# popgenmethods/smcpp

Measured on AMD Instinct MI355X. Metric: E-step loglik-evals/sec (100 Mbp, M=64, n=20), higher is better.
Workload: dtype f64 state + f32 scans (mixed)

## Files before the change

### smcpp_amd/csrc/engine_capi.hpp

```cpp
#define API_BEGIN try {
#define API_END                                                                    \
    return 0;                                                                      \
    }                                                                              \
    catch (const std::exception &e) { g_err = e.what(); return 1; }               \
    catch (...) { g_err = "unknown error"; return 1; }

extern "C" {

const char *smcpp_last_error(void) { return g_err.c_str(); }

int smcpp_create_onepop(int n, int n_contigs, const int *Ls, const int *const *obs, int n_hs, const double *hs,
                        double polarization_error, int device, smcpp_im **out) {
    API_BEGIN
    std::unique_ptr<smcpp_im> im(new smcpp_im());
    const int nn[1] = {n}, nna[1] = {2};
    im->build(1, nn, nna, n_contigs, Ls, obs, n_hs, hs, polarization_error, device);
    *out = im.release();
    API_END
}

int smcpp_create_twopop(int n1, int n2, int a1, int a2, int n_contigs, const int *Ls, const int *const *obs,
                        int n_hs, const double *hs, double polarization_error, int device, smcpp_im **out) {
    API_BEGIN
    if (a1 == 0 && a2 == 2) throw std::runtime_error("(0,2) not supported");
// ... 64 lines not shown
int smcpp_set_prep_mode(smcpp_im *im, int host) {
    API_BEGIN
    im->force_host_prep = host != 0;
    im->params_fresh = false;
    im->dirty = true;
    API_END
}

int smcpp_set_warm_start(smcpp_im *im, int on) {
    API_BEGIN
    im->warm_start = on != 0;
    if (!on) im->warm_valid = false;
    API_END
}

int smcpp_set_raw(smcpp_im *im, const double *pi, const double *T, int K, const int *keys, const double *E) {
    API_BEGIN
    const int M = im->M, kl = im->keylen;
    std::map<std::vector<int>, int> given;
    for (int k = 0; k < K; ++k) given[std::vector<int>(keys + (size_t)k * kl, keys + (size_t)(k + 1) * kl)] = k;
    std::vector<double> Enew((size_t)im->K * M);
    for (int k = 0; k < im->K; ++k) {
        std::vector<int> key(im->keys.begin() + (size_t)k * kl, im->keys.begin() + (size_t)(k + 1) * kl);
        auto it = given.find(key);
        if (it == given.end()) throw std::runtime_error("set_raw: an observed key has no emission vector");
        std::memcpy(&Enew[(size_t)k * M], E + (size_t)it->second * M, sizeof(double) * M);
    }
    im->pi.assign(pi, pi + M);
    im->T.assign(T, T + (size_t)M * M);
    im->E.swap(Enew);
    im->raw_keys.assign(keys, keys + (size_t)K * kl);
    im->raw_E.assign(E, E + (size_t)K * M);
    im->have_raw = true;
    im->E_on_dev = false;
    im->tgen_valid = false; im->dT_valid = true; im->T_lazy = false;
    im->dirty = true;
    im->nder = 0;
    API_END
}

int smcpp_estep(smcpp_im *im, int fb_only) {
    API_BEGIN
    (void)fb_only;
    im->estep();
    API_END
}

int smcpp_loglik(smcpp_im *im, double *out) {
    API_BEGIN
    std::memcpy(out, im->loglik.data(), sizeof(double) * im->n_contigs);
    API_END
}

static double dcs(const std::vector<double> &x) {
    if (x.empty()) return 0.0;
    double s = x[0], c = 0.0;
    for (size_t i = 1; i < x.size(); ++i) {
        const double y = c + x[i];
        const double u = x[i] - (y - c);
        const double t = y + s;
        const double v = y - (t - s);
        const double z = u + v;
        s = t + z;
        c = z - (s - t);
    }
    return s;
// ... 261 lines not shown
    return cols;
}
int smcpp_get_emission(smcpp_im *im, double *out, double *jac) {
    API_BEGIN
    need_model_params(im);
    im->sync_host_E();
    if (im->emission.size() != (size_t)im->M * smcpp_num_emission_cols(im)) throw std::runtime_error("emission matrix is not available");
    std::memcpy(out, im->emission.data(), sizeof(double) * im->emission.size());
    if (jac && im->nder > 0) std::memcpy(jac, im->demission.data(), sizeof(double) * im->demission.size());
    API_END
}

void smcpp_init_logger_cb(void (*cb)(const char *, const char *, const char *)) { g_logger_cb = cb; }

int smcpp_init_cache(const char *path) {
    API_BEGIN
    smcpp_host::csfs_cache_prefix() = path ? path : "";
    API_END
}

int smcpp_set_global_keys(smcpp_im *im, int Kg, const int *gkeys) {
    API_BEGIN
    const int kl = im->keylen;
    std::map<std::vector<int>, int> gm;
    for (int k = 0; k < Kg; ++k) gm[std::vector<int>(gkeys + (size_t)k * kl, gkeys + (size_t)(k + 1) * kl)] = k;
    im->local_to_global.assign(im->K, -1);
    for (int k = 0; k < im->K; ++k) {
        auto it = gm.find(std::vector<int>(im->keys.begin() + (size_t)k * kl, im->keys.begin() + (size_t)(k + 1) * kl));
        if (it == gm.end()) throw std::runtime_error("global key list misses a local key");
        im->local_to_global[k] = it->second;
    }
    im->gkeys.assign(gkeys, gkeys + (size_t)Kg * kl);
    im->have_global = true;
    im->pack_tables_ready = false;
    if (im->dprep) im->dprep->keys_ready = false;
    if (im->qdev) im->qdev->stats_ready = false;
    im->E_on_dev = false;
    im->params_fresh = false;
    im->Eg.clear(); im->dEg.clear();
    API_END
}

int smcpp_pack_stats(smcpp_im *im, double *buf, long *n_out, int dev) {
    API_BEGIN
    const int M = im->M, K = im->K;
    const int Kg = im->have_global ? (int)(im->gkeys.size() / im->keylen) : K;
    const long n = 1 + M + (long)M * M + (long)Kg * M;
    if (n_out) *n_out = n;
    if (!buf) return 0;
    if (dev && !im->estep_done) throw std::runtime_error("no E-step has been run on this manager yet");
    if (dev) {
        HIPCHK(hipSetDevice(im->device));
        if (!im->pack_tables_ready) {
            std::vector<int> g2l(Kg, -1);
            for (int k = 0; k < K; ++k) g2l[im->have_global ? im->local_to_global[k] : k] = k;
            im->d_g2l.upload(g2l, im->stream);
            im->d_present.upload(im->present, im->stream);
            HIPCHK(hipStreamSynchronize(im->stream));
            im->pack_tables_ready = true;
        }
        PackArgs pa;
        pa.M = M; pa.Mp = im->Mp; pa.K = K; pa.Kg = Kg; pa.n_contigs = im->n_contigs;
        pa.loglik = im->d_loglik.p; pa.gamma0 = im->d_gamma0.p; pa.xisum = im->d_xisum.p; pa.gsum = im->d_gsum.p;
        pa.present = im->d_present.p; pa.g2l = im->d_g2l.p; pa.out = buf;
        hipLaunchKernelGGL(k_pack_stats, dim3((unsigned)((n + 255) / 256)), dim3(256), 0, im->stream, pa);
        HIPCHK(hipGetLastError());
// ... 41 lines not shown
```

### smcpp_amd/csrc/engine_manager.hpp

```cpp
struct smcpp_im {
    int npop = 1, keylen = 3, M = 0, Mp = 0, NPL = 1, NT = 1, n_contigs = 0, K = 0, G = 0, Ke = 0;
    int n[2] = {0, 0}, na[2] = {2, 0};
    double polarization_error = 0.5;
    std::vector<double> hs;
    std::unique_ptr<smcpp_host::TwoPopPrep> twopop_prep;
    std::unique_ptr<TwoPopDevCsfs> twopop_dev;
    std::vector<int> keys;
    std::vector<int> Ls;
    std::vector<long long> contig_base;
    long long total_rows = 0;
    std::vector<RowInfo> rowinfo;
    std::vector<Group> groups;
    std::vector<int> eig_kid;
    std::vector<int> eig_of_key;
    std::vector<unsigned char> present;
    std::vector<double> span_sum;
    std::vector<double> pi_default;
    std::vector<unsigned char> key_nbpos;
    std::vector<Chunk> chunks;
    int max_chunks_per_contig = 1;
    int user_rows_per_chunk = 0;
    std::vector<int> perm1, perme;
    std::vector<int2> perm1k;
    std::vector<Slab> slabs_sc, slabs_rk, slabs_eg;
// ... 62 lines not shown
        size_t in_cap = 0;
        double *h_out = nullptr;
        size_t h_out_cap = 0;
        bool stats_ready = false;
        int Kq = 0;
        ~QDev() { if (d_in) (void)hipFree(d_in); if (h_out) (void)hipHostFree(h_out); }
    };
    std::unique_ptr<QDev> qdev;
    bool q_device(double val[4], double *jac);
    void ensure_dT();
    bool ss_static = false;
    bool ss_hybrid = false;
    bool ss_halo = false;
    int ss_hyb_th = 0x7fffffff;
    static constexpr int SS_HYB_COST = 8;
    long long ss_row_cost(int span) const { return (ss_hybrid && span > ss_hyb_th) ? SS_HYB_COST : span; }
    bool ss_dirsplit = false;
    int ss_nk_lds = 0, ss_ekey_of_slot[4] = {0, 1, 2, 3}, ss_eslot_of_key[4] = {0, 1, 2, 3};
    size_t ss_tab_bytes() const { return ss_hybrid ? ((size_t)ss_nk_lds * (ss_dirsplit ? 2 : 4) * Mp * (Mp + 1) + 8 * 64) * sizeof(double) : 0; }
    bool ss_active = false;
    bool eigfree = false;
    int ss_max_span = 0;
    int ss_nlds = 0;
    int ss_wpc = 1;
    bool ss_mid = false;
    int ss_wg_waves = 4;
    int ss_launched = 0, last_ss_passes = 0;
    bool ss_need_cert_pass = false;
    long long ss_positions = 0;
    int ss_light_f = 0, ss_light_b = 0;
    bool ss_warm_valid = false;
    bool arena_side = false;
    int ss_warm_parity = 0, ss_pass0 = 0;
    std::vector<int> ss_slot_of_key;
    DevBuf<int2> d_rowdesc_ss;
    bool split_spans = false;
    std::vector<int> user_Ls;
    std::vector<std::vector<int>> split_store, piece_row;
    std::vector<const int *> split_ptr;
    std::vector<DevBuf<int>> d_piece_first;
    DevBuf<double> d_gamma_user;
    const double *merged_gamma(int c);
    std::vector<GPiece> gp_pieces;
    std::vector<GTile> gp_tiles;
    std::vector<int> gp_pfirst;
    bool gp_built = false, gamma_pieces_last = false;
    DevBuf<GPiece> d_gp_pieces;
    DevBuf<GTile> d_gp_tiles;
    DevBuf<int> d_gp_pfirst;
    DevBuf<float> d_gp_pvf;
    DevBuf<double> d_gp_pvb, d_gp_pgam, d_gp_cs, d_gp_l2d, d_gp_gen;
    long long gp_count = -1;
    long long gamma_piece_count();
    void build_gamma_pieces();
    bool ss_generators_only();
    DevBuf<float> d_gpark;
    DevBuf<double> d_Fall;
    SsArgs ss_args;
    std::vector<Chunk> chunks_b;
    std::vector<int> ss_tasks;
    DevBuf<Chunk> d_chunks_b;
    DevBuf<int> d_tasks;
    void update_pi_default();
    bool debug = false;
    void upload_chunk_state();
    bool ss_extract_generators();
// ... 55 lines not shown
    int h_flags_cap = 0, h_ll_cap = 0;
    size_t param_cap = 0;
    int llblk = 64;
    int ZS = 8;
    int ZG = 1;
    int max_pass = 0;
    int last_fwd_passes = 0, last_bwd_passes = 0;
    float eps_f = 2e-6f;
    double eps_b = 1e-6;
    std::vector<double> loglik, h_xisum, h_gsum, h_gamma0;
    bool stats_on_host = false;
    double timing[9] = {0};
    double host_timing[4] = {0};
    std::vector<int> gkeys;
    std::vector<int> local_to_global;
    bool have_global = false;
    std::vector<double> g_stats;
    bool have_reduced = false;
    std::vector<double> Eg, dEg;
    std::vector<int> raw_keys;
    std::vector<double> raw_E;
    void global_emissions();

    ~smcpp_im() {
        if (stream) {
            for (auto &e : ev) (void)hipEventDestroy(e);
            (void)hipStreamDestroy(stream);
            if (stream2) (void)hipStreamDestroy(stream2);
            if (stream3) (void)hipStreamDestroy(stream3);
            if (stream_hi) (void)hipStreamDestroy(stream_hi);
        }
        if (d_param) (void)hipFree(d_param);
        if (d_pre) (void)hipFree(d_pre);
        if (h_flags) (void)hipHostFree(h_flags);
        if (h_ll) (void)hipHostFree(h_ll);
        if (h_done) (void)hipHostFree(h_done);
    }

    void build(int npop_, const int *nn, const int *nna, int n_contigs_, const int *Ls_, const int *const *obs,
               int n_hs, const double *hs_, double pol, int dev);
    void make_chunks();
    void make_slabs();
    void alloc_device();
    void host_prep_and_upload();
    void stage_static_and_prepass();
    void setup_power();
    ChainArgs chain_args();
    void run_chains();
    void run_stats();
    void enqueue_stats();
    void finish_stats();
    bool stats_enqueued = false;
    void estep();
    void fetch_stats();
    void prepare_params();
};

void smcpp_im::build(int npop_, const int *nn, const int *nna, int n_contigs_, const int *Ls_,
                     const int *const *obs, int n_hs, const double *hs_, double pol, int dev) {
    npop = npop_;
    keylen = 3 * npop;
    for (int p = 0; p < npop; ++p) { n[p] = nn[p]; na[p] = nna[p]; }
    polarization_error = pol;
    if (n_contigs_ <= 0) throw std::runtime_error("Observations list is empty");
    if (n_hs < 2) throw std::runtime_error("need at least two hidden state boundaries");
    hs.assign(hs_, hs_ + n_hs);
    for (int i = 1; i < n_hs; ++i)
        if (!(hs[i] >= hs[i - 1])) throw std::runtime_error("Hidden states must be in ascending order");
    M = n_hs - 1;
    Mp = (M + 15) / 16 * 16;
    NPL = M > 512 ? 16 : M > 256 ? 8 : (M + 63) / 64;
    NT = Mp / 16;
    if (M > 1024) throw std::runtime_error("M > 1024 hidden states is not supported by this build");
    n_contigs = n_contigs_;
    Ls.assign(Ls_, Ls_ + n_contigs);
    user_Ls = Ls;
    {
        const int ncol_ = 1 + keylen;
// ... 333 lines not shown
    long long rows = total_rows - n_contigs;
    int lc = user_rows_per_chunk;
    if (lc <= 0) {
        lc = opt().i(smcpp_opt::O_ROWS_PER_CHUNK, lc);
    }
    if (lc <= 0) lc = (int)std::max<long long>(512, (rows + slots - 1) / slots);
    chunks.clear();
    max_chunks_per_contig = 1;
    for (int c = 0; c < n_contigs; ++c) {
        const int L = Ls[c];
        const int nc = std::max(1, ceil_div(L, lc));
        max_chunks_per_contig = std::max(max_chunks_per_contig, nc);
        for (int j = 0; j < nc; ++j) {
            Chunk ch;
            ch.base = contig_base[c];
            ch.r0 = (int)((long long)L * j / nc);
            ch.r1 = (int)((long long)L * (j + 1) / nc);
            ch.contig = c;
            ch.first = (j == 0);
            ch.last = (j == nc - 1);
            ch.pad = 0;
            ch.h0 = ch.h1 = ch.r0;
            chunks.push_back(ch);
        }
    }
    max_pass = max_chunks_per_contig + 3;
    if (ss_static) max_pass += 4 + 2;
    chunks_b = chunks;
    for (Chunk &cb : chunks_b) cb.h0 = cb.h1 = cb.r1;
    ss_halo = false;
}

void smcpp_im::upload_chunk_state() {
    ss_warm_valid = false;
    const size_t nch = std::max(chunks.size(), chunks_b.size());
    d_chunks.upload(chunks, stream);
    d_chunks_b.upload(chunks_b, stream);
    {
        const size_t nf = chunks.size(), nb = chunks_b.size();
        ss_tasks.clear();
        size_t i = 0, j = 0;
        if (ss_hybrid && ss_dirsplit) {
            const size_t W = (size_t)ss_wg_waves;
            while (i < nf || j < nb) {
                const bool take_f = j >= nb || (i < nf && (double)i * (double)nb <= (double)j * (double)nf);
                for (size_t q = 0; q < W; ++q) {
                    if (take_f) ss_tasks.push_back(i < nf ? (int)i++ : -1);
                    else ss_tasks.push_back(j < nb ? ((1 << 30) | (int)j++) : -1);
                }
            }
        } else
        while (i < nf || j < nb) {
            const bool take_f = j >= nb || (i < nf && (double)i * (double)nb <= (double)j * (double)nf);
            if (take_f) ss_tasks.push_back((int)i++);
            else ss_tasks.push_back((1 << 30) | (int)j++);
        }
        while (ss_tasks.size() % ss_wg_waves) ss_tasks.push_back(-1);
        d_tasks.upload(ss_tasks, stream);
    }
    d_ends_f.alloc(2 * nch * Mp); d_used_f.alloc(nch * Mp);
    d_ends_b.alloc(2 * nch * Mp); d_used_b.alloc(nch * Mp);
    d_changed_f.alloc(max_pass + 1); d_changed_b.alloc(max_pass + 1);
    HIPCHK(hipStreamSynchronize(stream));
}

void smcpp_im::update_pi_default() {
    pi_default.assign(M, 0.0);
// ... 295 lines not shown
```

### smcpp_amd/csrc/engine_options.hpp

```cpp
#pragma once

namespace smcpp_opt {

enum OptId {
    O_HOST_TRACE, O_HOST_TIMING, O_OMP_BLOCKTIME, O_DUAL_STREAM, O_EVENT_FLAGS, O_LOCK_MIN_ROWS, O_CHAIN, O_SS, O_HYBRID, O_HYB_TH,
    O_COOP_BPC, O_ROWS_PER_CHUNK, O_SS_WPC, O_SS_HALO, O_HALO_LF, O_HALO_DF, O_HALO_LB, O_HALO_DB, O_SS_FWD_SHARE, O_STATS_TEAM,
    O_SLAB_ROWS, O_POWER_PREPASS, O_PREP, O_Q, O_EIG_TEAM, O_EIG_PIN, O_BWD_PRIO, O_COOP_TAB, O_POWER_DEBUG, O_BWD_PRIO_MASK,
    O_DEBUG_CYCLES, O_SS_H32, O_SS_MIXED, O_SS_LIGHT_F, O_SS_LIGHT_B, O_SS_CERT_PASS, O_POLL, O_SPEC_GAMMA, O_GAMMA_SIDE,
    O_STATS_VARIANT, O_SPAN_SCAN, O_S1_FUSE, O_EIGFREE, O_CSFS_DIRECT, O_RANK_WIDE, O_GAMMA_SCAN, O_GAMMA_PIECES, O_SPLIT_SPANS, O_T_LAZY, O_DEBUG_POISON, O_DEBUG_POISON_ONLY, O_DEBUG_POISON_LOG, O_COUNT
};

struct OptDef { const char *name, *help; };

static const OptDef OPT_DEFS[O_COUNT] = {
    {"SMCPP_HOST_TRACE",     "> 0: print a timestamped trace of the host phase of every E-step to stderr"},
    {"SMCPP_HOST_TIMING",    "set: print the split of the cold preparation / eigensolver / joint CSFS to stderr"},
    {"SMCPP_OMP_BLOCKTIME",  "libomp block time in ms (default 0; two-population managers 2)"},
    {"SMCPP_DUAL_STREAM",    "0: statistics branches on one stream"},
    {"SMCPP_EVENT_FLAGS",    "hipEventCreateWithFlags flags (default hipEventDisableSystemFence; 0 = default events)"},
    {"SMCPP_LOCK_MIN_ROWS",  "rows per (CU x 16) from which the lock-step MFMA chains are selected"},
    {"SMCPP_CHAIN",          "lock | dense | ss: force a chain family"},
    {"SMCPP_SS",             "0: no scan chains (the dense families)"},
    {"SMCPP_HYBRID",         "0: no hybrid rows on un-binned data (dense chains)"},
    {"SMCPP_HYB_TH",         "span above which a row is one eigen-power step (default 6)"},
    {"SMCPP_COOP_BPC",       "workgroups per CU of the cooperative chains"},
    {"SMCPP_ROWS_PER_CHUNK", "rows per chunk (0 = automatic)"},
    {"SMCPP_SS_WPC",         "wavefronts per SIMD of the scan chains (1..4; default by input size: M <= 64 two from 1.95, three from 12 million positions)"},
    {"SMCPP_SS_HALO",        "1 / 0: force / forbid the halo pass of the scan chains (default: M > 64, and M <= 64 with 1.35 - 12 million positions)"},
    {"SMCPP_HALO_LF",        "float halo positions, forward (2800)"},
    {"SMCPP_HALO_DF",        "exact halo positions, forward (800)"},
    {"SMCPP_HALO_LB",        "float halo positions, backward (3900)"},
    {"SMCPP_HALO_DB",        "exact halo positions, backward (1100)"},
    {"SMCPP_SS_FWD_SHARE",   "share of the wavefronts given to the forward chain"},
    {"SMCPP_STATS_TEAM",     "0: one rank partial per slab instead of per team of four"},
    {"SMCPP_SLAB_ROWS",      "minimum rows per statistics slab (128)"},
    {"SMCPP_POWER_PREPASS",  "0 / 1: eigen-free pre-pass of the dense chains off / forced"},
    {"SMCPP_PREP",           "host: the whole cold preparation on host threads"},
    {"SMCPP_Q",              "host: Q and its gradient on the host"},
    {"SMCPP_EIG_TEAM",       "threads per eigen key of the host eigensolver"},
    {"SMCPP_EIG_PIN",        "0: do not pin eigensolver teams to one L3 domain"},
    {"SMCPP_BWD_PRIO",       "s_setprio of the backward cooperative chain (0..3, default 1)"},
    {"SMCPP_COOP_TAB",       "0: test hook, tables of the cooperative chains from global memory"},
    {"SMCPP_POWER_DEBUG",    "debug level of the pre-pass"},
    {"SMCPP_BWD_PRIO_MASK",  "bit mask of the passes that raise the backward chain's priority (7)"},
    {"SMCPP_DEBUG_CYCLES",   "set: shader clocks / positions of chunk 1, pass 0 to stderr"},
    {"SMCPP_SS_H32",         "0: no two-row form of the scans at M <= 32"},
    {"SMCPP_SS_MIXED",       "0: fp64 scans in the stored passes; 1: float scans (default, one state per lane)"},
    {"SMCPP_SS_LIGHT_F",     "number of float history passes, forward"},
    {"SMCPP_SS_LIGHT_B",     "number of float history passes, backward"},
    {"SMCPP_SS_CERT_PASS",   "1: launch the all-skip certificate pass up front"},
    {"SMCPP_POLL",           "0: hipStreamSynchronize instead of polling the pinned completion word"},
    {"SMCPP_SPEC_GAMMA",     "0: save_gamma E-steps wait for the certificate before the statistics"},
    {"SMCPP_GAMMA_SIDE",     "0: per-row gammas on the main stream"},
    {"SMCPP_STATS_VARIANT",  "bit mask of stream arrangements of the statistics phase"},
    {"SMCPP_SPAN_SCAN",      "0: span fold on the matrix cores (k_span_big) instead of the scans"},
    {"SMCPP_S1_FUSE",        "0 / 1: two-kernel / one-pass span-1 statistics"},
    {"SMCPP_EIGFREE",        "0: eigensystem statistics even where the eigen-free form applies"},
    {"SMCPP_CSFS_DIRECT",    "set: literal O(pieces^2 n^2) conditioned SFS (test hook)"},
    {"SMCPP_RANK_WIDE",      "0: rank updates at M > 128 without the LDS-staged operand rows (k_rank_acc instead of k_rank_acc_wide); 4: four wavefronts per workgroup instead of eight"},
    {"SMCPP_GAMMA_SCAN",     "0: save_gamma E-steps take the eigensystem statistics and per-row gammas (M <= 256) instead of the eigen-free scans"},
    {"SMCPP_GAMMA_PIECES",   "0: per-row gammas of long rows at 64 < M <= 256 from the eigensystem (k_gamma_rows_eig) instead of eigen-power pieces + scan steps"},
    {"SMCPP_SPLIT_SPANS",    "0: rows of binned data longer than 64 positions are not cut into pieces (M > 64); 2: un-binned rows are cut as well at M <= 256 (test switch)"},
    {"SMCPP_T_LAZY",         "0: the model path expands the M x M transition matrix before the chains start and takes their generators from it (rounds 3-5)"},
    {"SMCPP_DEBUG_POISON",   "byte value every fresh device allocation is filled with (255: NaN / -1): a kernel that reads memory it was "
                             "never given shows up as NaN in a fresh process instead of depending on what the allocator recycles"},
    {"SMCPP_DEBUG_POISON_ONLY", "poison only the allocation with this index (counted from the last smcpp_reload_options): tools/poison_probe.py"},
    {"SMCPP_DEBUG_POISON_LOG",  "set: print index, source line and size of every device allocation to stderr"},
};

struct EngineOptions {
    bool set_[O_COUNT];
    std::string val_[O_COUNT];
    long long ival_[O_COUNT];
    double dval_[O_COUNT];
    unsigned generation = 0;
    void parse() {
        for (int k = 0; k < O_COUNT; ++k) {
            const char *e = getenv(OPT_DEFS[k].name);
            set_[k] = e != nullptr;
            val_[k] = e ? e : "";
            ival_[k] = e ? strtoll(e, nullptr, 0) : 0;
            dval_[k] = e ? atof(e) : 0.0;
        }
// ... 48 lines not shown
```

### smcpp_amd/csrc/engine_plans.hpp

```cpp
template <int MT_, bool TAB_, bool RERUN_, bool HOT2_>
static void launch_chain_coop2_tt(bool fwd, const ChainArgs &a, const CoopArgs &ca, size_t shm, hipStream_t s) {
    if (fwd) {
        static bool once = false;
        if (!once) { HIPCHK(hipFuncSetAttribute((const void *)k_fwd_coop2<MT_, TAB_, RERUN_, HOT2_>, hipFuncAttributeMaxDynamicSharedMemorySize, 160 * 1024)); once = true; }
        hipLaunchKernelGGL((k_fwd_coop2<MT_, TAB_, RERUN_, HOT2_>), dim3(a.nchunks), dim3(MT_ * 4), shm, s, a, ca);
    } else {
        static bool once = false;
        if (!once) { HIPCHK(hipFuncSetAttribute((const void *)k_bwd_coop2<MT_, TAB_, RERUN_, HOT2_>, hipFuncAttributeMaxDynamicSharedMemorySize, 160 * 1024)); once = true; }
        hipLaunchKernelGGL((k_bwd_coop2<MT_, TAB_, RERUN_, HOT2_>), dim3(a.nchunks), dim3(MT_ * 4), shm, s, a, ca);
    }
}
template <int MT_, bool TAB_>
static void launch_chain_power_t(bool fwd, const ChainArgs &a, const CoopArgs &ca, size_t shm, hipStream_t s) {
    if (fwd) {
        static bool once = false;
        if (!once) { HIPCHK(hipFuncSetAttribute((const void *)k_fwd_coop2<MT_, TAB_, false, false, true>, hipFuncAttributeMaxDynamicSharedMemorySize, 160 * 1024)); once = true; }
        hipLaunchKernelGGL((k_fwd_coop2<MT_, TAB_, false, false, true>), dim3(a.nchunks), dim3(MT_ * 4), shm, s, a, ca);
    } else {
        static bool once = false;
        if (!once) { HIPCHK(hipFuncSetAttribute((const void *)k_bwd_coop2<MT_, TAB_, false, false, true>, hipFuncAttributeMaxDynamicSharedMemorySize, 160 * 1024)); once = true; }
        hipLaunchKernelGGL((k_bwd_coop2<MT_, TAB_, false, false, true>), dim3(a.nchunks), dim3(MT_ * 4), shm, s, a, ca);
    }
}
template <int MT_, bool TAB_, bool RERUN_>
// ... 459 lines not shown
template <int NPL_, bool HYB_>
static void launch_chain_ss_t(const SsArgs &a, int ntasks, size_t shm, hipStream_t s, int wgw) {
    const bool h32_off = opt().off(smcpp_opt::O_SS_H32);
    if (NPL_ == 1 && !HYB_ && a.K <= a.nlds && a.Mp <= 32 && !h32_off) launch_chain_ss_tt<NPL_, HYB_, true, NPL_ == 1 && !HYB_>(a, ntasks, shm, s, wgw);
    else if (a.K <= a.nlds) launch_chain_ss_tt<NPL_, HYB_, true>(a, ntasks, shm, s, wgw);
    else launch_chain_ss_tt<NPL_, HYB_, false>(a, ntasks, shm, s, wgw);
}
static void launch_chain_ss(int npl, const SsArgs &a, int ntasks, size_t shm, hipStream_t s, int wgw = 4) {
    switch (npl) {
        case 1: if (a.hyb_th != 0x7fffffff) launch_chain_ss_t<1, true>(a, ntasks, shm, s, wgw); else launch_chain_ss_t<1, false>(a, ntasks, shm, s, 4); break;
        case 2: launch_chain_ss_t<2, false>(a, ntasks, shm, s, 4); break;
        case 3: launch_chain_ss_t<3, false>(a, ntasks, shm, s, 4); break;
        case 4: launch_chain_ss_t<4, false>(a, ntasks, shm, s, 4); break;
        case 8: launch_chain_ss_t<8, false>(a, ntasks, shm, s, 4); break;
        case 16: launch_chain_ss_t<16, false>(a, ntasks, shm, s, 4); break;
        default: throw std::runtime_error("unsupported number of hidden states");
    }
}


void smcpp_im::ss_launch_passes(int upto) {
    const size_t shm = (size_t)ss_nlds * 64 * NPL * sizeof(double) + ss_tab_bytes();
    for (; ss_launched < upto; ++ss_launched) {
        const int p = ss_launched;
        const bool lf = p < ss_light_f, lb = p < ss_light_b;
        ss_args.pass = p;
        ss_args.mode_f = lf ? 2 : p == 0 ? 0 : 1;
        ss_args.mode_b = lb ? 2 : p == 0 ? 0 : 1;
        ss_args.full_f = (p > 0 && p == ss_light_f) ? 1 : 0;
        ss_args.full_b = (p > 0 && p == ss_light_b) ? 1 : 0;
        launch_chain_ss(NPL, ss_args, (int)ss_tasks.size(), shm, stream, ss_wg_waves);
    }
    HIPCHK(hipGetLastError());
}

void smcpp_im::ss_launch_initial() {
    hipStream_t s = stream;
    const int MS = 64 * NPL;
    std::vector<float> &pi_f = hs_pi_f;
    if (pi_f.size() != (size_t)Mp) pi_f.assign(Mp, 0.f);
    for (int i = 0; i < M; ++i) pi_f[i] = (float)pi[i];
    const size_t need = 12 * 256 + pi_f.size() * 4 + ss_gen.size() * 8 + (size_t)K * MS * 8;
    pre_stage.reset(need);
    if (need > pre_cap) {
        if (d_pre) (void)hipFree(d_pre);
        pre_cap = need + need / 4;
        HIPCHK(hipMalloc((void **)&d_pre, pre_cap));
        smcpp_opt::poison(d_pre, pre_cap, __LINE__, __FILE__);
    }
    size_t off = 0;
    auto put = [&](const void *src, size_t bytes) {
        off = (off + 255) & ~(size_t)255;
        if (src) std::memcpy(pre_stage.base + off, src, bytes);
        char *dp = d_pre + off;
        off += bytes;
        return dp;
    };
    SsArgs &a = ss_args;
    a = SsArgs();
    a.M = M; a.Mp = Mp; a.nchunks = (int)chunks.size(); a.pass = 0; a.K = K; a.nlds = ss_nlds;
    a.chunks = d_chunks.p; a.rowdesc = d_rowdesc_ss.p + ROWDESC_PAD;
    a.chunks_b = d_chunks_b.p; a.nchunks_b = (int)chunks_b.size(); a.tasks = d_tasks.p;
    a.pi_f = reinterpret_cast<const float *>(put(pi_f.data(), pi_f.size() * 4));
    const double *gd = reinterpret_cast<const double *>(put(ss_gen.data(), ss_gen.size() * 8));
    a.f_dc = gd; a.f_g = gd + MS; a.f_cg = gd + 2 * MS; a.f_b = gd + 3 * MS; a.f_a = gd + 4 * MS; a.f_d = gd + 5 * MS;
    a.b_dc = gd + 6 * MS; a.b_g = gd + 7 * MS; a.b_b = gd + 8 * MS; a.b_a = gd + 9 * MS;
    a.c0 = ss_c0;
    if (E_on_dev) a.E = dprep->d_Es.p;
    else {
        const size_t eoff = (off + 255) & ~(size_t)255;
        double *he = reinterpret_cast<double *>(pre_stage.base + eoff);
        std::memset(he, 0, (size_t)K * MS * 8);
        for (int k = 0; k < K; ++k)
            std::memcpy(he + (size_t)ss_slot_of_key[k] * MS, &E[(size_t)k * M], sizeof(double) * M);
        a.E = reinterpret_cast<const double *>(put(nullptr, (size_t)K * MS * 8));
    }
    a.alpha = d_alpha.p; a.beta = d_beta.p; a.cnorm = d_cnorm.p;
    a.ends_f = d_ends_f.p; a.used_f = d_used_f.p; a.ends_b = d_ends_b.p; a.used_b = d_used_b.p;
    {
        if (h_flags_cap < 4 * (max_pass + 1)) {
            if (h_flags) (void)hipHostFree(h_flags);
            h_flags_cap = 4 * (max_pass + 1);
            HIPCHK(hipHostMalloc((void **)&h_flags, sizeof(int) * h_flags_cap, hipHostMallocCoherent | hipHostMallocMapped));
            d_flags_view = nullptr;
        }
        if (!d_flags_view) HIPCHK(hipHostGetDevicePointer((void **)&d_flags_view, h_flags, 0));
        if (!h_done) {
            HIPCHK(hipHostMalloc((void **)&h_done, 64, hipHostMallocCoherent | hipHostMallocMapped));
            *h_done = 0;
            HIPCHK(hipHostGetDevicePointer((void **)&d_done_view, h_done, 0));
        }
        std::memset(h_flags, 0, sizeof(int) * h_flags_cap);
    }
    a.changed_f = d_flags_view; a.changed_b = d_flags_view + (max_pass + 1);
    a.endchg_f = d_flags_view + 2 * (max_pass + 1); a.endchg_b = d_flags_view + 3 * (max_pass + 1);
    a.eps_f = eps_f; a.eps_b = eps_b; a.full_f = a.full_b = 0;
    {
        const bool mixed_on = !opt().off(smcpp_opt::O_SS_MIXED);
        a.mixed = (mixed_on && NPL == 1 && !ss_hybrid) ? 1 : 0;
    }
    if (ss_hybrid) {
        a.hyb_th = ss_hyb_th; a.Ke = Ke; a.hot_ek = std::max(0, hot_eig); a.dirsplit = ss_dirsplit ? 1 : 0;
        a.nk_lds = ss_nk_lds;
        for (int e = 0; e < 4; ++e) { a.key_of_slot[e] = ss_ekey_of_slot[e]; a.slot_of_key[e] = ss_eslot_of_key[e]; }
        a.Pinvrm = d_Pinvrm.p; a.Prm = d_Prm.p; a.PinvT = d_PinvT.p; a.PT = d_PT.p; a.dsc = d_dsc.p;
    }
    {
        long long pos = 0;
        const int ef = opt().i(smcpp_opt::O_SS_LIGHT_F, -1), eb = opt().i(smcpp_opt::O_SS_LIGHT_B, -1);
        pos = ss_positions / std::max<size_t>(1, chunks.size());
        const long long pos_b = ss_positions / std::max<size_t>(1, chunks_b.size());
        auto pick = [&](double hist, long long p_) { return p_ <= 0 || (double)p_ > 1.5 * hist ? 0 : std::min(4, (int)std::ceil(hist / (double)p_)); };
        ss_light_f = ef >= 0 ? ef : pick(2800.0, pos);
        ss_light_b = eb >= 0 ? eb : pick(3900.0, pos_b);
        if (chunks.size() <= (size_t)n_contigs) ss_light_f = 0;
        if (chunks_b.size() <= (size_t)n_contigs) ss_light_b = 0;
    }
    if (ss_hybrid) ss_light_f = ss_light_b = 0;
    const bool use_halo = ss_halo && !(warm_start && ss_warm_valid) && chunks.size() > (size_t)n_contigs && chunks_b.size() > (size_t)n_contigs;
    if (use_halo) ss_light_f = ss_light_b = 0;
    a.halo = use_halo ? 1 : 0;
    ss_pass0 = 0;
    if (warm_start && ss_warm_valid && chunks.size() > (size_t)n_contigs && chunks_b.size() > (size_t)n_contigs) {
        ss_pass0 = ss_warm_parity == 0 ? 1 : 2;
        ss_light_f = ss_pass0 + std::max(0, ss_light_f - 1);
        ss_light_b = ss_pass0 + std::max(0, ss_light_b - 1);
    }
    ss_warm_valid = false;
    a.dbg = nullptr;
    if (opt().has(smcpp_opt::O_DEBUG_CYCLES)) { d_dbg.alloc(16); d_dbg.zero(s); a.dbg = d_dbg.p; }
    HIPCHK(hipMemcpyAsync(d_pre, pre_stage.base, off, hipMemcpyHostToDevice, s));
    HIPCHK(hipEventRecord(ev[10], s));
    ss_launched = ss_pass0;
    const bool cert_launch = opt().on(smcpp_opt::O_SS_CERT_PASS);
    const int want = std::min(max_pass, std::max(ss_pass0 + (last_ss_passes > 0 ? last_ss_passes + (cert_launch || ss_need_cert_pass ? 1 : 0) : 6),
                                                 std::max(ss_light_f, ss_light_b) + 2));
    ss_launch_passes(want);
}

bool smcpp_im::wait_done(int epoch) {
    const auto t0 = std::chrono::steady_clock::now();
    unsigned n = 0;
    while (__atomic_load_n(h_done, __ATOMIC_ACQUIRE) != epoch) {
#if defined(__x86_64__) || defined(__i386__)
        __builtin_ia32_pause();
#else
        std::this_thread::yield();
#endif
        if ((++n & 0x3fff) == 0 && std::chrono::duration<double>(std::chrono::steady_clock::now() - t0).count() > 5.0) {
            HIPCHK(hipStreamSynchronize(stream));
            return __atomic_load_n(h_done, __ATOMIC_ACQUIRE) == epoch;
        }
    }
    return true;
}

void smcpp_im::run_chains_ss() {
    hipStream_t s = stream;
    const int *chf = h_flags, *chb = h_flags + (max_pass + 1);
    const int p0 = ss_pass0;
    auto first_quiet = [p0](const int *cf, const int *cb, int upto) {
        for (int j = p0; j < upto; ++j)
            if (cf[j] == 0 && cb[j] == 0) return j;
        return -1;
    };
    ss_warm_valid = false;
// ... 11 lines not shown
        } else stats_enqueued = false;
        done_covers_stats = stats_enqueued;
        if (poll) {
            ++done_epoch;
            if (!done_folded) hipLaunchKernelGGL(k_signal, dim3(1), dim3(1), 0, s, d_done_view, done_epoch);
            if (!wait_done(done_epoch)) throw std::runtime_error("the device did not signal completion");
        } else HIPCHK(hipStreamSynchronize(s));
        first_round = false;
        q = first_quiet(chf, chb, ss_launched);
        if (q < 0 && ss_launched > p0) {
            const int L = ss_launched - 1;
            const int *ecf = h_flags + 2 * (max_pass + 1), *ecb = h_flags + 3 * (max_pass + 1);
            if (ecf[L] == 0 && ecb[L] == 0) q = ss_launched;
        }
        if (q >= 0 || ss_launched >= max_pass) break;
        stats_enqueued = false;
        done_covers_stats = false;
        if (first_launched < 0) first_launched = ss_launched;
        ss_launch_passes(std::min(max_pass, ss_launched + 3));
    }
    chains_dual = false;
    if (ss_args.dbg) {
        long long h[8];
        HIPCHK(hipMemcpy(h, d_dbg.p, sizeof(h), hipMemcpyDeviceToHost));
        fprintf(stderr, "[cycles] ss pass 0, chunk 1: forward %lld shader clocks, %lld x 10 ns, %lld positions, %lld rows; backward %lld "
                "clocks, %lld x 10 ns, %lld positions, %lld rows\n", h[0], h[1], h[2], h[3], h[4], h[5], h[6], h[7]);
    }
    if (q < 0) { stats_enqueued = false; throw std::runtime_error("chunk-boundary iteration did not converge"); }
    if (first_launched >= 0 && q == first_launched) ss_need_cert_pass = true;
    last_ss_passes = q - p0;
    last_fwd_passes = last_bwd_passes = q - p0;
    ss_warm_parity = (ss_launched - 1) & 1;
    ss_warm_valid = true;
}

void smcpp_im::run_stats() {
    if (!stats_enqueued) enqueue_stats();
    finish_stats();
}

void smcpp_im::finish_stats() {
    if (!(ss_active && done_covers_stats)) HIPCHK(hipStreamSynchronize(stream));
    done_covers_stats = false;
    std::memcpy(loglik.data(), h_ll, sizeof(double) * n_contigs);
    stats_enqueued = false;
}

void smcpp_im::enqueue_stats() {
    hipStream_t s = stream;
    if (h_ll_cap < n_contigs) {
        if (h_ll) (void)hipHostFree(h_ll);
        h_ll_cap = n_contigs;
        HIPCHK(hipHostMalloc((void **)&h_ll, sizeof(double) * h_ll_cap, hipHostMallocCoherent | hipHostMallocMapped));
        HIPCHK(hipHostGetDevicePointer((void **)&d_ll_view, h_ll, 0));
    }
    if (arena_side) HIPCHK(hipStreamWaitEvent(s, ev[20], 0));
    auto arena_wait = [&](hipStream_t x) { if (arena_side && x != s) HIPCHK(hipStreamWaitEvent(x, ev[20], 0)); };
    LoglikArgs la;
    la.cnorm = d_cnorm.p; la.rowinfo = d_rowinfo.p; la.g_logscale = d_g_logscale.p;
    la.contig_base = d_contig_base.p; la.contig_L = d_contig_L.p; la.partial = d_llpart.p; la.loglik = d_loglik.p;
    la.logc = d_logc.p; la.nblk = llblk;
    la.loglik_host = d_ll_view;
    const bool gamma_pieces = save_gamma && n_e_rows > 0 && !eigfree && NT > 4 && Mp <= 256 && !opt().off(smcpp_opt::O_GAMMA_PIECES) &&
                              (double)gamma_piece_count() * Mp * 20.0 < 96e9 && (ss_active || ss_generators_only());
    const bool gamma_side = save_gamma && n_e_rows > 0 && dual_stream && stream_hi != nullptr && !gamma_pieces &&
                            !opt().off(smcpp_opt::O_GAMMA_SIDE);
// ... 416 lines not shown
        (void)hipEventElapsedTime(&b_ms, ev[2], ev[3]);
    } else {
        (void)hipEventElapsedTime(&f_ms, ev[1], ev[2]);
        (void)hipEventElapsedTime(&b_ms, ev[2], ev[3]);
    }
    float chains_ms = 0;
    if (ss_active) {
        (void)hipEventElapsedTime(&chains_ms, ev[10], ev[3]);
        f_ms = b_ms = chains_ms;
    } else (void)hipEventElapsedTime(&chains_ms, ev[1], ev[3]);
    if (prepass_launched) {
        (void)hipEventElapsedTime(&pre_f_ms, ev[10], ev[11]);
        (void)hipEventElapsedTime(&pre_b_ms, ev[12], ev[13]);
        f_ms += pre_f_ms; b_ms += pre_b_ms;
        chains_ms += std::max(pre_f_ms, pre_b_ms);
    }
    (void)hipEventElapsedTime(&s_ms, ev[3], ev[4]);
    (void)hipEventElapsedTime(&fin_ms, ev[4], ev[5]);
    (void)hipGetLastError();
    timing[0] = t_host01;
    timing[1] = chains_ms;
    timing[2] = f_ms; timing[3] = b_ms; timing[4] = s_ms; timing[5] = fin_ms;
    timing[6] = t_host12;
    timing[7] = last_fwd_passes; timing[8] = last_bwd_passes;
}

void smcpp_im::estep() {
    if (std::isnan(theta) || std::isnan(rho) || std::isnan(alpha))
        throw std::runtime_error("theta / rho / alpha must be set");
    HIPCHK(hipSetDevice(device));
    timing_pending = false;
    auto t0 = std::chrono::steady_clock::now();
    HostTrace tr;
    prepare_params();
    tr.mark("estep: prepare_params");
    host_timing[0] = std::chrono::duration<double, std::milli>(std::chrono::steady_clock::now() - t0).count();
    if ((int)pi.size() != M || (!T_lazy && (int)T.size() != M * M) || (!E_on_dev && (int)E.size() != K * M))
        throw std::runtime_error("parameters are not set");
    HIPCHK(hipEventRecord(ev[0], stream));
    const bool eigfree_off = opt().off(smcpp_opt::O_EIGFREE);
    const bool gamma_scan = !opt().off(smcpp_opt::O_GAMMA_SCAN);
    const bool eigfree_static = !eigfree_off && Mp <= 1024 && ss_max_span <= 64 && (!save_gamma || gamma_scan);
    if (Mp > 256 && !(ss_static && eigfree_static))
        throw std::runtime_error("more than 256 hidden states: only the scan chains with eigen-free statistics are built (rows longer than "
                                 "64 positions are cut into pieces at construction unless SMCPP_SPLIT_SPANS=0 / SMCPP_EIGFREE=0 forbid it or "
                                 "the pieces would not fit the device)");
    if (E_on_dev && !(ss_static && eigfree_static)) sync_host_E();
    ss_active = ss_static && ss_extract_generators();
    if (Mp > 256 && !ss_active)
        throw std::runtime_error("more than 256 hidden states: the transition matrix must have the structure of the reference's "
                                 "HJTransition (the dense fallback kernels stop at 256)");
    tr.mark("estep: extract generators");
    if (!ss_active) ss_warm_valid = false;
    eigfree = ss_active && eigfree_static;
    if (E_on_dev && !(ss_active && eigfree)) sync_host_E();
    if (ss_active && !ss_hybrid) { prepass_launched = false; static_packed = false; ss_launch_initial(); }
    else if (ss_active) { prepass_launched = false; static_packed = false; }
    else stage_static_and_prepass();
    tr.mark("estep: first launches");
    host_prep_and_upload();
    tr.mark("estep: host_prep_and_upload");
    if (ss_active && ss_hybrid) ss_launch_initial();
    auto t1 = std::chrono::steady_clock::now();
    if (ss_active) run_chains_ss(); else run_chains();
    tr.mark("estep: chains (host view)");
    run_stats();
    tr.mark("estep: statistics enqueued");
    if (E_on_dev) {
        dprep->check_flags();
        if (ss_active && dprep->flags()[2]) {
            sync_host_E();
            estep();
            return;
        }
    }
    auto t2 = std::chrono::steady_clock::now();
    t_host01 = std::chrono::duration<double, std::milli>(t1 - t0).count();
    t_host12 = std::chrono::duration<double, std::milli>(t2 - t1).count();
    host_timing[3] = t_host01;
    timing_pending = true;
    if (g_logger_cb) {
        resolve_timing();
        log_msg("DEBUG", "E-step: %d contig(s), %lld rows, M = %d, K = %d keys; host %.3f ms, chains %.3f ms (%d forward / %d "
                "backward passes), statistics %.3f ms; loglik[0] = %.10g", n_contigs, total_rows - n_contigs, M, K, timing[0],
                timing[1], last_fwd_passes, last_bwd_passes, timing[4] + timing[5], loglik.empty() ? 0.0 : loglik[0]);
    }
    stats_on_host = false;
    have_reduced = false;
    if (qdev) qdev->stats_ready = false;
    gamma_valid = save_gamma;
    estep_done = true;
    dirty = false;
}

void smcpp_im::fetch_stats() {
    if (stats_on_host) return;
    if (!estep_done) {
        h_xisum.assign((size_t)n_contigs * M * M, 0.0);
// ... 31 lines not shown
```

### smcpp_amd/csrc/engine_rccl.hpp

```cpp
extern "C" {
struct ncclUniqueIdBlob { char b[128]; };
static void check_rc(int rc) { if (rc) throw std::runtime_error(g_err); }
struct RcclDirect {
    void *lib = nullptr;
    void *comm = nullptr;
    int world = 1, rank = 0;
    int (*get_uid)(void *) = nullptr;
    int (*init_rank)(void **, int, ncclUniqueIdBlob, int) = nullptr;
    int (*all_reduce)(const void *, void *, size_t, int, int, void *, hipStream_t) = nullptr;
    int (*destroy)(void *) = nullptr;
    const char *(*err_string)(int) = nullptr;
    DevBuf<double> buf;
    long n = 0;
    double *h_val = nullptr, *d_val_view = nullptr;
    int *h_flag = nullptr, *d_flag_view = nullptr;
    int epoch = 0;
    bool reduced_in_buf = false;
};
static void *rccl_handle(const char *libpath) {
    static std::mutex mu;
    static std::map<std::string, void *> handles;
    const std::string key = libpath && *libpath ? libpath : "librccl.so.1";
    std::lock_guard<std::mutex> lk(mu);
    auto it = handles.find(key);
// ... 127 lines not shown
        im->last_fwd_passes = im->last_bwd_passes = 0;
    }
    API_END
}

int smcpp_last_timing(smcpp_im *im, double out[9]) {
    API_BEGIN im->resolve_timing(); std::memcpy(out, im->timing, sizeof(double) * 9); API_END
}

int smcpp_last_host_timing(smcpp_im *im, double out[4]) {
    API_BEGIN std::memcpy(out, im->host_timing, sizeof(double) * 4); API_END
}

void *smcpp_stream(smcpp_im *im) { return (void *)im->stream; }

int smcpp_host_chunk_counts(int n_contigs, const long long *cost, const int *rows, long long nslots, long long floor_cost, int *out) {
    API_BEGIN
    if (n_contigs <= 0 || nslots <= 0) throw std::runtime_error("smcpp_host_chunk_counts: empty input");
    const std::vector<long long> c(cost, cost + n_contigs);
    const std::vector<int> r(rows, rows + n_contigs);
    const std::vector<int> ncs = ss_chunk_counts(c, r, nslots, floor_cost);
    std::copy(ncs.begin(), ncs.end(), out);
    API_END
}

int smcpp_chain_mode(smcpp_im *im) { return im ? (im->ss_static ? (im->ss_hybrid ? 6 : 5) : im->chain_mode) : -1; }

void smcpp_reload_options(void) { smcpp_opt::reload(); }

int smcpp_describe(smcpp_im *im, char *buf, int cap) {
    std::string s = "{";
    s += smcpp_opt::describe_options();
    if (im) {
        char t[1024];
        const int fam = im->ss_static ? (im->ss_hybrid ? 6 : 5) : im->chain_mode;
        snprintf(t, sizeof t,
                 ", \"plan\": {\"chain_family\": %d, \"scan_chains\": %s, \"hybrid_rows\": %s, \"states\": %d, \"states_padded\": %d, "
                 "\"states_per_lane\": %d, \"keys\": %d, \"eigen_keys\": %d, \"rows\": %lld, \"positions\": %lld, \"max_span\": %d, "
                 "\"chunks_forward\": %zu, \"chunks_backward\": %zu, \"wavefronts_per_simd\": %d, \"halo_pass\": %s, "
                 "\"light_passes_forward\": %d, \"light_passes_backward\": %d, \"float_scans_in_stored_passes\": %s, "
                 "\"passes_to_certificate\": %d, \"passes_launched\": %d, \"certificate_pass_launched_up_front\": %s, "
                 "\"save_gamma\": %s, \"eigen_free_statistics\": %s, \"per_row_gamma\": \"%s\", \"long_rows_cut\": %s, \"warm_start\": %s, \"host_threads\": %d}",
                 fam, im->ss_static ? "true" : "false", im->ss_hybrid ? "true" : "false", im->M, im->Mp, im->NPL, im->K, im->Ke,
                 (long long)(im->total_rows - im->n_contigs), (long long)im->ss_positions, im->ss_max_span, im->chunks.size(),
                 im->chunks_b.size(), im->ss_wpc, (im->ss_static && im->ss_args.halo) ? "true" : "false", im->ss_light_f, im->ss_light_b,
                 (im->ss_static && im->ss_args.mixed) ? "true" : "false", im->last_ss_passes, im->ss_launched,
                 (opt().on(smcpp_opt::O_SS_CERT_PASS) || im->ss_need_cert_pass) ? "true" : "false", im->save_gamma ? "true" : "false",
                 im->eigfree ? "true" : "false", !im->save_gamma ? "none" : im->eigfree ? "scan steps" : im->gamma_pieces_last ? "eigen-power pieces + scan steps" : "eigensystem", im->split_spans ? "true" : "false",
                 im->warm_start ? "true" : "false", omp_get_max_threads());
        s += t;
    }
    s += "}";
    if (buf && cap > 0) {
        const size_t n = std::min(s.size(), (size_t)cap - 1);
        std::memcpy(buf, s.data(), n);
        buf[n] = 0;
    }
    return (int)s.size();
}

static int ss_debug_apply(int M, const double *T, int nvec, const double *x, const double *e, double *out_f, double *out_b, int float_scans);
int smcpp_debug_ss_apply(int M, const double *T, int nvec, const double *x, const double *e, double *out_f, double *out_b) {
    API_BEGIN
    return ss_debug_apply(M, T, nvec, x, e, out_f, out_b, 0);
    API_END
}
int smcpp_debug_ss_apply_float_scans(int M, const double *T, int nvec, const double *x, const double *e, double *out_f, double *out_b) {
    API_BEGIN
    if (M > 64) throw std::runtime_error("the all-float scans hold one state per lane: M <= 64");
    return ss_debug_apply(M, T, nvec, x, e, out_f, out_b, 1);
    API_END
}
static int ss_debug_apply(int M, const double *T, int nvec, const double *x, const double *e, double *out_f, double *out_b, int float_scans) {
    {
    const int NPL = M > 512 ? 16 : M > 256 ? 8 : (M + 63) / 64, MS = 64 * NPL;
    if (M > 1024) throw std::runtime_error("unsupported number of hidden states");
    std::vector<double> gen;
    double c0 = 0.0;
    if (!ss_generators(M, MS, T, gen, c0)) return 2;
    std::vector<double> hx((size_t)nvec * MS, 0.0), he((size_t)nvec * MS, 0.0);
// ... 51 lines not shown
```

Baseline: 1097.

## Launch speculative first light scan pass on anchor parameters during host prep

At the start of each E-step, the first float light pass of the scan chains is launched on a second stream, using a snapshot (anchor) of the previous E-step's precomputed device parameters and emissions. This lets GPU work overlap the host-side parameter preparation that previously had to finish before pass 0 could start. The main pass sequence then waits on the speculative pass and counts it as pass 1, relying on later passes to correct any difference from the new parameters. It adds a device-to-device snapshot copy per anchor, extra join points and invalidation logic, and the risk of extra passes when the parameters change a lot between E-steps.

```diff
diff --git a/smcpp_amd/csrc/engine_capi.hpp b/smcpp_amd/csrc/engine_capi.hpp
--- a/smcpp_amd/csrc/engine_capi.hpp
+++ b/smcpp_amd/csrc/engine_capi.hpp
@@ -120,6 +120,7 @@
     im->raw_keys.assign(keys, keys + (size_t)K * kl);
     im->raw_E.assign(E, E + (size_t)K * M);
     im->have_raw = true;
+    im->ss_spec_valid = false;
     im->E_on_dev = false;
     im->tgen_valid = false; im->dT_valid = true; im->T_lazy = false;
     im->dirty = true;
@@ -447,6 +448,7 @@
     }
     im->gkeys.assign(gkeys, gkeys + (size_t)Kg * kl);
     im->have_global = true;
+    im->ss_spec_valid = false;
     im->pack_tables_ready = false;
     if (im->dprep) im->dprep->keys_ready = false;
     if (im->qdev) im->qdev->stats_ready = false;
diff --git a/smcpp_amd/csrc/engine_manager.hpp b/smcpp_amd/csrc/engine_manager.hpp
--- a/smcpp_amd/csrc/engine_manager.hpp
+++ b/smcpp_amd/csrc/engine_manager.hpp
@@ -118,6 +118,13 @@
     bool ss_warm_valid = false;
     bool arena_side = false;
     int ss_warm_parity = 0, ss_pass0 = 0;
+    bool ss_spec_valid = false;
+    bool ss_spec_launched = false;
+    bool ss_spec_last = false;
+    char *d_anchor = nullptr;
+    size_t anchor_cap = 0, pre_used = 0;
+    SsArgs ss_anchor;
+    long long ss_spec_count = 0;
     std::vector<int> ss_slot_of_key;
     DevBuf<int2> d_rowdesc_ss;
     bool split_spans = false;
@@ -239,6 +246,7 @@
         }
         if (d_param) (void)hipFree(d_param);
         if (d_pre) (void)hipFree(d_pre);
+        if (d_anchor) (void)hipFree(d_anchor);
         if (h_flags) (void)hipHostFree(h_flags);
         if (h_ll) (void)hipHostFree(h_ll);
         if (h_done) (void)hipHostFree(h_done);
@@ -251,6 +259,9 @@
     void alloc_device();
     void host_prep_and_upload();
     void stage_static_and_prepass();
+    bool ss_launch_spec();
+    void ss_spec_join();
+    void ss_set_anchor();
     void setup_power();
     ChainArgs chain_args();
     void run_chains();
@@ -650,7 +661,9 @@
 }
 
 void smcpp_im::upload_chunk_state() {
+    ss_spec_join();
     ss_warm_valid = false;
+    ss_spec_valid = false;
     const size_t nch = std::max(chunks.size(), chunks_b.size());
     d_chunks.upload(chunks, stream);
     d_chunks_b.upload(chunks_b, stream);
diff --git a/smcpp_amd/csrc/engine_options.hpp b/smcpp_amd/csrc/engine_options.hpp
--- a/smcpp_amd/csrc/engine_options.hpp
+++ b/smcpp_amd/csrc/engine_options.hpp
@@ -6,7 +6,7 @@
     O_HOST_TRACE, O_HOST_TIMING, O_OMP_BLOCKTIME, O_DUAL_STREAM, O_EVENT_FLAGS, O_LOCK_MIN_ROWS, O_CHAIN, O_SS, O_HYBRID, O_HYB_TH,
     O_COOP_BPC, O_ROWS_PER_CHUNK, O_SS_WPC, O_SS_HALO, O_HALO_LF, O_HALO_DF, O_HALO_LB, O_HALO_DB, O_SS_FWD_SHARE, O_STATS_TEAM,
     O_SLAB_ROWS, O_POWER_PREPASS, O_PREP, O_Q, O_EIG_TEAM, O_EIG_PIN, O_BWD_PRIO, O_COOP_TAB, O_POWER_DEBUG, O_BWD_PRIO_MASK,
-    O_DEBUG_CYCLES, O_SS_H32, O_SS_MIXED, O_SS_LIGHT_F, O_SS_LIGHT_B, O_SS_CERT_PASS, O_POLL, O_SPEC_GAMMA, O_GAMMA_SIDE,
+    O_DEBUG_CYCLES, O_SS_H32, O_SS_MIXED, O_SS_LIGHT_F, O_SS_LIGHT_B, O_SS_CERT_PASS, O_SS_SPEC, O_POLL, O_SPEC_GAMMA, O_GAMMA_SIDE,
     O_STATS_VARIANT, O_SPAN_SCAN, O_S1_FUSE, O_EIGFREE, O_CSFS_DIRECT, O_RANK_WIDE, O_GAMMA_SCAN, O_GAMMA_PIECES, O_SPLIT_SPANS, O_T_LAZY, O_DEBUG_POISON, O_DEBUG_POISON_ONLY, O_DEBUG_POISON_LOG, O_COUNT
 };
 
@@ -49,6 +49,7 @@
     {"SMCPP_SS_LIGHT_F",     "number of float history passes, forward"},
     {"SMCPP_SS_LIGHT_B",     "number of float history passes, backward"},
     {"SMCPP_SS_CERT_PASS",   "1: launch the all-skip certificate pass up front"},
+    {"SMCPP_SS_SPEC",        "0: the first light pass of the scan chains waits for the host phase of the E-step instead of starting at its head on the anchor parameters"},
     {"SMCPP_POLL",           "0: hipStreamSynchronize instead of polling the pinned completion word"},
     {"SMCPP_SPEC_GAMMA",     "0: save_gamma E-steps wait for the certificate before the statistics"},
     {"SMCPP_GAMMA_SIDE",     "0: per-row gammas on the main stream"},
diff --git a/smcpp_amd/csrc/engine_plans.hpp b/smcpp_amd/csrc/engine_plans.hpp
--- a/smcpp_amd/csrc/engine_plans.hpp
+++ b/smcpp_amd/csrc/engine_plans.hpp
@@ -515,6 +515,59 @@
         launch_chain_ss(NPL, ss_args, (int)ss_tasks.size(), shm, stream, ss_wg_waves);
     }
     HIPCHK(hipGetLastError());
+}
+
+bool smcpp_im::ss_launch_spec() {
+    ss_spec_launched = false;
+    const bool ok = ss_spec_valid && ss_static && !ss_hybrid && !have_raw && !warm_start && stream2 && h_flags && !ss_args.dbg &&
+                    !opt().off(smcpp_opt::O_SS_SPEC);
+    if (!ok) return false;
+    std::memset(h_flags, 0, sizeof(int) * h_flags_cap);
+    HIPCHK(hipEventRecord(ev[18], stream));
+    HIPCHK(hipStreamWaitEvent(stream2, ev[18], 0));
+    HIPCHK(hipEventRecord(ev[10], stream2));
+    SsArgs a = ss_args;
+    a.pi_f = ss_anchor.pi_f; a.c0 = ss_anchor.c0; a.E = ss_anchor.E;
+    a.f_dc = ss_anchor.f_dc; a.f_g = ss_anchor.f_g; a.f_cg = ss_anchor.f_cg; a.f_b = ss_anchor.f_b; a.f_a = ss_anchor.f_a;
+    a.f_d = ss_anchor.f_d; a.b_dc = ss_anchor.b_dc; a.b_g = ss_anchor.b_g; a.b_b = ss_anchor.b_b; a.b_a = ss_anchor.b_a;
+    a.pass = 0; a.mode_f = a.mode_b = 2; a.full_f = a.full_b = 0;
+    const size_t shm = (size_t)ss_nlds * 64 * NPL * sizeof(double) + ss_tab_bytes();
+    launch_chain_ss(NPL, a, (int)ss_tasks.size(), shm, stream2, ss_wg_waves);
+    HIPCHK(hipGetLastError());
+    HIPCHK(hipEventRecord(ev[21], stream2));
+    ss_spec_launched = true;
+    ++ss_spec_count;
+    return true;
+}
+
+void smcpp_im::ss_spec_join() {
+    if (!ss_spec_launched) return;
+    HIPCHK(hipEventSynchronize(ev[21]));
+    ss_spec_launched = false;
+    std::memset(h_flags, 0, sizeof(int) * h_flags_cap);
+}
+
+void smcpp_im::ss_set_anchor() {
+    const bool e_dev = E_on_dev;
+    const size_t ebytes = e_dev ? dprep->d_Es.n * sizeof(double) : 0;
+    const size_t eoff = (pre_used + 255) & ~(size_t)255, need = eoff + ebytes;
+    if (need > anchor_cap) {
+        if (d_anchor) (void)hipFree(d_anchor);
+        anchor_cap = need;
+        HIPCHK(hipMalloc((void **)&d_anchor, anchor_cap));
+        smcpp_opt::poison(d_anchor, anchor_cap, __LINE__, __FILE__);
+    }
+    HIPCHK(hipMemcpyAsync(d_anchor, d_pre, pre_used, hipMemcpyDeviceToDevice, stream));
+    if (ebytes) HIPCHK(hipMemcpyAsync(d_anchor + eoff, ss_args.E, ebytes, hipMemcpyDeviceToDevice, stream));
+    auto rebase = [&](const auto *p) { return reinterpret_cast<decltype(p)>(d_anchor + (reinterpret_cast<const char *>(p) - d_pre)); };
+    SsArgs &an = ss_anchor;
+    an = ss_args;
+    an.pi_f = rebase(ss_args.pi_f);
+    an.f_dc = rebase(ss_args.f_dc); an.f_g = rebase(ss_args.f_g); an.f_cg = rebase(ss_args.f_cg); an.f_b = rebase(ss_args.f_b);
+    an.f_a = rebase(ss_args.f_a); an.f_d = rebase(ss_args.f_d); an.b_dc = rebase(ss_args.b_dc); an.b_g = rebase(ss_args.b_g);
+    an.b_b = rebase(ss_args.b_b); an.b_a = rebase(ss_args.b_a);
+    an.E = e_dev ? reinterpret_cast<const double *>(d_anchor + eoff) : rebase(ss_args.E);
+    ss_spec_valid = true;
 }
 
 void smcpp_im::ss_launch_initial() {
@@ -562,6 +615,7 @@
     a.ends_f = d_ends_f.p; a.used_f = d_used_f.p; a.ends_b = d_ends_b.p; a.used_b = d_used_b.p;
     {
         if (h_flags_cap < 4 * (max_pass + 1)) {
+            ss_spec_join();
             if (h_flags) (void)hipHostFree(h_flags);
             h_flags_cap = 4 * (max_pass + 1);
             HIPCHK(hipHostMalloc((void **)&h_flags, sizeof(int) * h_flags_cap, hipHostMallocCoherent | hipHostMallocMapped));
@@ -573,7 +627,7 @@
             *h_done = 0;
             HIPCHK(hipHostGetDevicePointer((void **)&d_done_view, h_done, 0));
         }
-        std::memset(h_flags, 0, sizeof(int) * h_flags_cap);
+        if (!ss_spec_launched) std::memset(h_flags, 0, sizeof(int) * h_flags_cap);
     }
     a.changed_f = d_flags_view; a.changed_b = d_flags_view + (max_pass + 1);
     a.endchg_f = d_flags_view + 2 * (max_pass + 1); a.endchg_b = d_flags_view + 3 * (max_pass + 1);
@@ -610,11 +664,14 @@
         ss_light_b = ss_pass0 + std::max(0, ss_light_b - 1);
     }
     ss_warm_valid = false;
+    if (ss_spec_launched && !(ss_pass0 == 0 && !use_halo && ss_light_f > 0 && ss_light_b > 0)) ss_spec_join();
     a.dbg = nullptr;
-    if (opt().has(smcpp_opt::O_DEBUG_CYCLES)) { d_dbg.alloc(16); d_dbg.zero(s); a.dbg = d_dbg.p; }
+    if (opt().has(smcpp_opt::O_DEBUG_CYCLES)) { ss_spec_join(); d_dbg.alloc(16); d_dbg.zero(s); a.dbg = d_dbg.p; }
     HIPCHK(hipMemcpyAsync(d_pre, pre_stage.base, off, hipMemcpyHostToDevice, s));
-    HIPCHK(hipEventRecord(ev[10], s));
-    ss_launched = ss_pass0;
+    pre_used = off;
+    if (!ss_spec_launched) HIPCHK(hipEventRecord(ev[10], s));
+    ss_launched = ss_spec_launched ? 1 : ss_pass0;
+    if (ss_spec_launched) HIPCHK(hipStreamWaitEvent(s, ev[21], 0));
     const bool cert_launch = opt().on(smcpp_opt::O_SS_CERT_PASS);
     const int want = std::min(max_pass, std::max(ss_pass0 + (last_ss_passes > 0 ? last_ss_passes + (cert_launch || ss_need_cert_pass ? 1 : 0) : 6),
                                                  std::max(ss_light_f, ss_light_b) + 2));
@@ -692,6 +749,9 @@
     last_fwd_passes = last_bwd_passes = q - p0;
     ss_warm_parity = (ss_launched - 1) & 1;
     ss_warm_valid = true;
+    if (!ss_spec_valid && !ss_hybrid && !have_raw && !warm_start && ss_pass0 == 0 && !ss_args.halo && ss_light_f > 0 && ss_light_b > 0 &&
+        !ss_args.dbg && !opt().off(smcpp_opt::O_SS_SPEC))
+        ss_set_anchor();
 }
 
 void smcpp_im::run_stats() {
@@ -1174,6 +1234,8 @@
     timing_pending = false;
     auto t0 = std::chrono::steady_clock::now();
     HostTrace tr;
+    ss_launch_spec();
+    tr.mark("estep: speculative pass 0");
     prepare_params();
     tr.mark("estep: prepare_params");
     host_timing[0] = std::chrono::duration<double, std::milli>(std::chrono::steady_clock::now() - t0).count();
@@ -1194,6 +1256,7 @@
                                  "HJTransition (the dense fallback kernels stop at 256)");
     tr.mark("estep: extract generators");
     if (!ss_active) ss_warm_valid = false;
+    if (!ss_active || ss_hybrid) { ss_spec_join(); ss_spec_valid = false; }
     eigfree = ss_active && eigfree_static;
     if (E_on_dev && !(ss_active && eigfree)) sync_host_E();
     if (ss_active && !ss_hybrid) { prepass_launched = false; static_packed = false; ss_launch_initial(); }
@@ -1206,6 +1269,8 @@
     auto t1 = std::chrono::steady_clock::now();
     if (ss_active) run_chains_ss(); else run_chains();
     tr.mark("estep: chains (host view)");
+    ss_spec_last = ss_active && ss_spec_launched;
+    ss_spec_launched = false;
     run_stats();
     tr.mark("estep: statistics enqueued");
     if (E_on_dev) {
diff --git a/smcpp_amd/csrc/engine_rccl.hpp b/smcpp_amd/csrc/engine_rccl.hpp
--- a/smcpp_amd/csrc/engine_rccl.hpp
+++ b/smcpp_amd/csrc/engine_rccl.hpp
@@ -183,7 +183,7 @@
     std::string s = "{";
     s += smcpp_opt::describe_options();
     if (im) {
-        char t[1024];
+        char t[1536];
         const int fam = im->ss_static ? (im->ss_hybrid ? 6 : 5) : im->chain_mode;
         snprintf(t, sizeof t,
                  ", \"plan\": {\"chain_family\": %d, \"scan_chains\": %s, \"hybrid_rows\": %s, \"states\": %d, \"states_padded\": %d, "
@@ -191,12 +191,14 @@
                  "\"chunks_forward\": %zu, \"chunks_backward\": %zu, \"wavefronts_per_simd\": %d, \"halo_pass\": %s, "
                  "\"light_passes_forward\": %d, \"light_passes_backward\": %d, \"float_scans_in_stored_passes\": %s, "
                  "\"passes_to_certificate\": %d, \"passes_launched\": %d, \"certificate_pass_launched_up_front\": %s, "
+                 "\"speculative_pass_0\": %s, \"speculative_pass_0_count\": %lld, "
                  "\"save_gamma\": %s, \"eigen_free_statistics\": %s, \"per_row_gamma\": \"%s\", \"long_rows_cut\": %s, \"warm_start\": %s, \"host_threads\": %d}",
                  fam, im->ss_static ? "true" : "false", im->ss_hybrid ? "true" : "false", im->M, im->Mp, im->NPL, im->K, im->Ke,
                  (long long)(im->total_rows - im->n_contigs), (long long)im->ss_positions, im->ss_max_span, im->chunks.size(),
                  im->chunks_b.size(), im->ss_wpc, (im->ss_static && im->ss_args.halo) ? "true" : "false", im->ss_light_f, im->ss_light_b,
                  (im->ss_static && im->ss_args.mixed) ? "true" : "false", im->last_ss_passes, im->ss_launched,
-                 (opt().on(smcpp_opt::O_SS_CERT_PASS) || im->ss_need_cert_pass) ? "true" : "false", im->save_gamma ? "true" : "false",
+                 (opt().on(smcpp_opt::O_SS_CERT_PASS) || im->ss_need_cert_pass) ? "true" : "false",
+                 im->ss_spec_last ? "true" : "false", im->ss_spec_count, im->save_gamma ? "true" : "false",
                  im->eigfree ? "true" : "false", !im->save_gamma ? "none" : im->eigfree ? "scan steps" : im->gamma_pieces_last ? "eigen-power pieces + scan steps" : "eigensystem", im->split_spans ? "true" : "false",
                  im->warm_start ? "true" : "false", omp_get_max_threads());
         s += t;
```

Measured after the change: 1158 (median of 6 runs). 1.06x the previous value.
